# OettlM/STEDM

Hardware: AMD Instinct MI355X
Metric: U-Net denoising steps/sec (32x32x4 latent, bs=64) (higher is better)
Workload: dtype f16; 1 GPU; HER2-style DDIM-50 + CFG 1.5 (rescale 0.7) denoising step, NS32 U-Net (234.6M params, random-init PRNG weights), 32x32x4 latents + 3-ch layout concat, style vector 512; batch_per_gpu=64, global_batch=64, latent=32x32x4, cfg=cond+uncond per step, parallelism=dp1 (independent latents, no in-loop collective)

## Files before the change

include/stedm_hip.h:

```cpp
#ifndef STEDM_HIP_H
#define STEDM_HIP_H

#include <stdint.h>

#ifdef __cplusplus
extern "C" {
#endif

#define STEDM_ABI_VERSION 18

#define STEDM_F16 0
#define STEDM_BF16 1

#define STEDM_CONV_S1 0
#define STEDM_CONV_DOWN 1
#define STEDM_CONV_UP 2
#define STEDM_CONV_UP_SUBPIXEL 3
#define STEDM_CONV_S2D 4

int stedm_abi_version(void);
const char* stedm_last_error(void);
int stedm_device_cus(void);

#define STEDM_F16G_RAW 1
#define STEDM_F16G_NORM 2
#define STEDM_F16G_CONV_OUT16 4
#define STEDM_F16G_S2D 8
#define STEDM_F16G_CAST 16
#define STEDM_F16G_CONV_SRC 32
int stedm_f16_guard_set(void* flag_words);

int stedm_pack_conv_weight(const float* w_oihw, void* w_hi, void* w_lo, int cout, int cin, int ks,
                           int mm_dtype, void* stream);
int stedm_pack_conv_weight_up(const float* w_oihw, void* w_hi, void* w_lo, int cout, int cin, int mm_dtype,
                              void* stream);
int stedm_pack_conv_weight_frag(const float* w_oihw, void* out, int cout, int cin, int ks, int mm_dtype, void* stream);
int stedm_pack_conv_weight_up_frag(const float* w_oihw, void* out, int cout, int cin, int mm_dtype, void* stream);
int stedm_space_to_depth16(const float* x, int C, int B, int H, int W, void* out_hi, void* out_lo, int mm_dtype, void* stream);
int stedm_pack_conv_weight_frag16(const float* w, long sn, long sc, int flip, void* out, int cout, int cin, int ks, int mm_dtype, void* stream);
int stedm_pack_conv_weight_frag16_hl(const float* w, long sn, long sc, int flip, void* out, int cout, int cin, int mm_dtype, void* stream);
int stedm_pack_conv_weight_frag16_hl1(const float* w, long sn, long sc, int flip, void* out, int cout, int cin, int mm_dtype, void* stream);
int stedm_pack_conv_weight_up_frag16_hl(const float* w, void* out, int cout, int cin, int mm_dtype, void* stream);
int stedm_pack_conv_weight_s2d_frag16_hl(const float* w, void* out, int cout, int cin, int mm_dtype, int pad_br, void* stream);
int stedm_pack_conv_weight_s2d_frag(const float* w_oihw, void* out, int cout, int cin, int mm_dtype, int pad_br, void* stream);
int stedm_transpose_f32(const float* in, float* out, int rows, int cols, void* stream);

int stedm_gn_scale_shift(const float* x1, int c1, const float* x2, int c2, int x2_bmod,
                         const float* gamma, const float* beta, float eps, int groups, int B, int HW,
                         float* scale, float* shift, void* stream);

int stedm_gn_nslab(int C, int HW);
int stedm_gn_chan_nslab(int HW);
int stedm_gn_chan_stats(const float* x, int C, int B, int HW, int nslab, float* chan_stats, void* stream);
int stedm_gn_chan_stats16(const float* x, int C, int B, int HW, int nslab, float* chan_stats, void* out_hi, void* out_lo, int mm_dtype,
                          void* stream);
int stedm_gn_apply16c(const float* x1, int c1, const float* cs1, int nslab1, const float* x2, int c2, const float* cs2, int nslab2, int x2_bmod,
                      const float* gamma, const float* beta, float eps, int groups, int act, int B, int HW,
                      void* out_hi, void* out_lo, void* raw_hi, void* raw_lo, int mm_dtype, void* stream);
int stedm_gn_apply16c_mr(const float* x1, int c1, const float* cs1, int nslab1, const float* x2, int c2, const float* cs2, int nslab2, int x2_bmod,
                         const float* gamma, const float* beta, float eps, int groups, int act, int B, int HW,
                         void* out_hi, void* out_lo, void* raw_hi, void* raw_lo, float* mean_rstd, int mm_dtype, void* stream);
int stedm_gn_apply16c_x16(int c1, const float* cs1, int nslab1, const float* x2, int c2, const float* cs2, int nslab2, int x2_bmod,
                          const float* gamma, const float* beta, float eps, int groups, int act, int B, int HW,
                          void* out_hi, void* raw_hi, int mm_dtype, void* stream);
int stedm_gn_stats(const float* x1, int c1, const float* x2, int c2, int x2_bmod, int groups, int B, int HW,
                   double* stats, void* stream);
int stedm_gn_apply16(const float* x1, int c1, const float* x2, int c2, int x2_bmod, const float* gamma,
                     const float* beta, float eps, int groups, int act, const double* stats, int B, int HW,
                     void* out_hi, void* out_lo, int mm_dtype, void* stream);

typedef struct stedm_conv_args {
  const float* src1;
  const float* src2;
  int32_t c1, c2, src2_bmod;
  int32_t B, Hin, Win;
  int32_t mode;
  int32_t ks;
  const float* scale;
  const float* shift;
  int32_t act;
  const void* w_hi;
  const void* w_lo;
  const float* bias;
  const float* emb;
  int32_t emb_bstride;
  const float* res;
  float* out;
  int32_t cout;
  int32_t npass;
  int32_t mm_dtype;
  const void* src16_hi;
  const void* src16_lo;
  int32_t act_out;
  void* out16_hi;
  void* out16_lo;
  const void* w_frag;
  float* chan_stats;
  const void* src16b_hi;
  const void* w_frag_b;
  const float* bias_b;
  int32_t cb;
  float* ws;
  int64_t ws_floats;
  int32_t chan_nslab;
  const void* w_frag16;
  const void* w_frag_b16;
  int32_t pad_br;
  const float* gn_gamma;
  const float* gn_beta;
  float gn_eps;
  int32_t gn_groups;
  int32_t gn_act;
  void* gn_out16;
  float* gn_mr;
  int32_t gn_only;
  void* gn_out16_lo;
  void* qkv_q;
// ... 198 lines not shown
```

stedm_amd/_lib.py:

```python
from __future__ import annotations

import ctypes as C
import os

_HERE = os.path.dirname(os.path.abspath(__file__))
LIB_PATH = os.environ.get("STEDM_HIP_LIB") or os.path.join(_HERE, "libstedm_hip.so")

ABI_VERSION = 18
F16, BF16 = 0, 1
CONV_S1, CONV_DOWN, CONV_UP, CONV_UP_SUBPIXEL, CONV_S2D = 0, 1, 2, 3, 4


class StedmHipError(RuntimeError):
    pass


class ConvArgs(C.Structure):
    _fields_ = [
        ("src1", C.c_void_p), ("src2", C.c_void_p),
        ("c1", C.c_int32), ("c2", C.c_int32), ("src2_bmod", C.c_int32),
        ("B", C.c_int32), ("Hin", C.c_int32), ("Win", C.c_int32),
        ("mode", C.c_int32), ("ks", C.c_int32),
        ("scale", C.c_void_p), ("shift", C.c_void_p),
        ("act", C.c_int32),
        ("w_hi", C.c_void_p), ("w_lo", C.c_void_p), ("bias", C.c_void_p),
        ("emb", C.c_void_p), ("emb_bstride", C.c_int32),
        ("res", C.c_void_p), ("out", C.c_void_p),
        ("cout", C.c_int32), ("npass", C.c_int32), ("mm_dtype", C.c_int32),
        ("src16_hi", C.c_void_p), ("src16_lo", C.c_void_p),
        ("act_out", C.c_int32), ("out16_hi", C.c_void_p), ("out16_lo", C.c_void_p),
        ("w_frag", C.c_void_p), ("chan_stats", C.c_void_p),
        ("src16b_hi", C.c_void_p), ("w_frag_b", C.c_void_p), ("bias_b", C.c_void_p), ("cb", C.c_int32),
        ("ws", C.c_void_p), ("ws_floats", C.c_int64), ("chan_nslab", C.c_int32), ("w_frag16", C.c_void_p), ("w_frag_b16", C.c_void_p), ("pad_br", C.c_int32),
        ("gn_gamma", C.c_void_p), ("gn_beta", C.c_void_p), ("gn_eps", C.c_float), ("gn_groups", C.c_int32), ("gn_act", C.c_int32), ("gn_out16", C.c_void_p), ("gn_mr", C.c_void_p), ("gn_only", C.c_int32),
        ("gn_out16_lo", C.c_void_p),
        ("qkv_q", C.c_void_p), ("qkv_k", C.c_void_p), ("qkv_vt", C.c_void_p),
        ("qkv_T", C.c_int32), ("qkv_Tp", C.c_int32), ("qkv_heads", C.c_int32), ("qkv_qscale", C.c_float),
        ("ln_gamma", C.c_void_p), ("ln_beta", C.c_void_p), ("ln_res", C.c_void_p), ("ln_eps", C.c_float),
        ("out16_stride", C.c_int32),
        ("gn_coop", C.c_void_p), ("gn_coop_epoch", C.c_void_p), ("gn_coop_tmo", C.c_void_p),
    ]


_P, _I, _F = C.c_void_p, C.c_int, C.c_float
SIGNATURES = {
    "stedm_abi_version": (_I, []),
    "stedm_last_error": (C.c_char_p, []),
    "stedm_device_cus": (_I, []),
    "stedm_f16_guard_set": (_I, [_P]),
    "stedm_pack_conv_weight": (_I, [_P, _P, _P, _I, _I, _I, _I, _P]),
    "stedm_pack_conv_weight_up": (_I, [_P, _P, _P, _I, _I, _I, _P]),
    "stedm_pack_conv_weight_frag": (_I, [_P, _P, _I, _I, _I, _I, _P]),
    "stedm_pack_conv_weight_up_frag": (_I, [_P, _P, _I, _I, _I, _P]),
    "stedm_pack_conv_weight_frag16": (_I, [_P, C.c_long, C.c_long, _I, _P, _I, _I, _I, _I, _P]),
    "stedm_pack_conv_weight_frag16_hl": (_I, [_P, C.c_long, C.c_long, _I, _P, _I, _I, _I, _P]),
    "stedm_pack_conv_weight_frag16_hl1": (_I, [_P, C.c_long, C.c_long, _I, _P, _I, _I, _I, _P]),
    "stedm_pack_conv_weight_up_frag16_hl": (_I, [_P, _P, _I, _I, _I, _P]),
    "stedm_pack_conv_weight_s2d_frag16_hl": (_I, [_P, _P, _I, _I, _I, _I, _P]),
    "stedm_pack_conv_weight_s2d_frag": (_I, [_P, _P, _I, _I, _I, _I, _P]),
    "stedm_space_to_depth16": (_I, [_P, _I, _I, _I, _I, _P, _P, _I, _P]),
    "stedm_transpose_f32": (_I, [_P, _P, _I, _I, _P]),
    "stedm_gn_scale_shift": (_I, [_P, _I, _P, _I, _I, _P, _P, _F, _I, _I, _I, _P, _P, _P]),
    "stedm_gn_nslab": (_I, [_I, _I]),
    "stedm_gn_stats": (_I, [_P, _I, _P, _I, _I, _I, _I, _I, _P, _P]),
    "stedm_gn_apply16": (_I, [_P, _I, _P, _I, _I, _P, _P, _F, _I, _I, _P, _I, _I, _P, _P, _I, _P]),
    "stedm_gn_chan_nslab": (_I, [_I]),
    "stedm_gn_chan_stats": (_I, [_P, _I, _I, _I, _I, _P, _P]),
    "stedm_gn_chan_stats16": (_I, [_P, _I, _I, _I, _I, _P, _P, _P, _I, _P]),
    "stedm_gn_apply16c": (_I, [_P, _I, _P, _I, _P, _I, _P, _I, _I, _P, _P, _F, _I, _I, _I, _I, _P, _P, _P, _P, _I, _P]),
    "stedm_gn_apply16c_mr": (_I, [_P, _I, _P, _I, _P, _I, _P, _I, _I, _P, _P, _F, _I, _I, _I, _I, _P, _P, _P, _P, _P, _I, _P]),
    "stedm_conv3x3_tiles_ok": (_I, [_I, _I]),
    "stedm_im2col_rows16": (_I, [_P, _P, _I, _I, _I, _I, _I, _P]),
    "stedm_philox_normal": (_I, [_P, _I, _I, _P, _I, C.c_ulonglong, C.c_uint, _P]),
    "stedm_ddim_mask_blend": (_I, [_P, _P, _P, C.c_long, C.c_long, _P, _P, _P, _P, _P, _I, _I, _I, C.c_long, C.c_ulonglong, _P]),
    "stedm_ddpm_step": (_I, [_P, _P, _P, _P, _I, _I, _P, _P, C.c_long, C.c_long, _P, _P, _P, _P, _I, _I, _I, C.c_long,
                            C.c_ulonglong, C.c_ulonglong, _P]),
    "stedm_gn_apply16c_x16": (_I, [_I, _P, _I, _P, _I, _P, _I, _I, _P, _P, _F, _I, _I, _I, _I, _P, _P, _I, _P]),
    "stedm_conv_igemm": (_I, [C.POINTER(ConvArgs), _P]),
    "stedm_conv_fused_skip_ok": (_I, [C.POINTER(ConvArgs)]),
    "stedm_conv_rs_ok": (_I, [C.POINTER(ConvArgs)]),
    "stedm_conv_in": (_I, [_P, _I, _P, _I, _I, _P, _P, _P, _I, _I, _I, _I, _P, _P]),
    "stedm_conv_out": (_I, [_P, _I, _P, _I, _P, _P, _F, _I, _P, _P, _P, _I, _I, _I, _I, _P]),
    "stedm_time_embed": (_I, [_P, _P, _P, _P, _P, _P, _P, _P, _I, _I, _I, _P]),
    "stedm_time_embed_f32": (_I, [_P, _P, _P, _P, _P, _P, _P, _P, _I, _I, _I, _P]),
    "stedm_emb_proj": (_I, [_P, _P, _P, _P, _I, _I, _I, _P]),
    "stedm_linear": (_I, [_P, _P, _P, _P, _I, _I, _I, _I, _I, _P]),
    "stedm_attn_legacy": (_I, [_P, _P, _I, _I, _I, _I, _P]),
    "stedm_attn_legacy16": (_I, [_P, _I, _P, _I, _I, _I, _I, _I, _P]),
    "stedm_ddim_step": (_I, [_P, _P, _P, _P, _P, _P, _F, _F, _P, _P, _I, _I, _I, _I, _P]),
    "stedm_ddim_step_ex": (_I, [_P, _P, _P, _P, _P, _P, _I, _F, _F, _I, _F, _F, C.c_long, C.c_ulonglong, _P, _P, _P, _P, _I, _I, _I, _I,
                               _P]),
    "stedm_step_advance": (_I, [_P, _I, _P]),
    "stedm_step_set_t": (_I, [_P, _P, _P, _I, _P]),
    "stedm_step_set_t_f32": (_I, [_P, _P, _P, _I, _P]),
    "stedm_dpm_step": (_I, [_P, _P, _P, _P, _P, _P, _P, _F, C.c_long, _P]),
    "stedm_dpm_update": (_I, [_P, _P, _P, _P, _P, C.c_long, _P, _P, _P, _F, _I, C.c_long, _P]),
    "stedm_dpm_threshold": (_I, [_P, C.c_long, _P, _P, _F, _I, C.c_long, _P, _P]),
    "stedm_plms_step": (_I, [_P, _P, _P, _P, _P, _P, _I, _I, _F, _P, _P, C.c_long, _P]),
    "stedm_svit_patch_embed": (_I, [_P, _I, _I, _I, _I, _I, _P, _P, _F, _P, _P, _P, _P, _P, _I, _P]),
    "stedm_svit_patch_ln16": (_I, [_P, _I, _I, _I, _I, _I, _P, _P, _F, _P, _P, _I, _P]),
    "stedm_svit_tok_place": (_I, [_P, _P, _P, _P, _I, _I, _I, _P]),
    "stedm_ln_apply16": (_I, [_P, _P, _P, _F, _P, _P, C.c_long, _I, _I, _P]),
    "stedm_qkv_pack": (_I, [_P, _I, _F, _P, _P, _P, _P, _P, _P, _I, _I, _I, _I, _I, _P]),
    "stedm_lsa_flash": (_I, [_P, _P, _P, _P, _P, _P, _P, _P, _I, _I, _I, _I, _I, _I, _P]),
    "stedm_lsa_flash_drop": (_I, [_P, _P, _P, _P, _P, _P, _P, _P, _I, _I, _I, _I, _I, _I, _F, C.c_ulonglong, C.c_uint, _P]),
    "stedm_dropout_rows": (_I, [_P, _P, _P, _P, _P, C.c_long, _F, C.c_ulonglong, C.c_uint, _I, _P]),
    "stedm_qkv_pack_mx8": (_I, [_P, _I, _F, _P, _P, _P, _P, _P, _P, _I, _I, _I, _I, _I, _P]),
    "stedm_lsa_flash_mx8": (_I, [_P, _P, _P, _P, _P, _P, _P, _I, _I, _I, _I, _I, _P]),
    "stedm_svit_head": (_I, [_P, _I, _I, _I, _I, _P, _P, _P, _F, _P, _P, _P, _I, _P, C.c_long, _P]),
    "stedm_ln_bwd_blocks": (_I, [C.c_long]),
    "stedm_ln_bwd": (_I, [_P, _P, _P, _F, _P, _P, _P, _P, _P, C.c_long, _I, _I, _P]),
    "stedm_geglu_bwd": (_I, [_P, _P, _P, C.c_long, _I, _P]),
    "stedm_geglu16": (_I, [_P, _P, _P, C.c_long, _I, _I, _P]),
    "stedm_agg_reduce": (_I, [_P, _P, _I, _I, _I, _I, _P]),
    "stedm_spatial_rescale": (_I, [_P, _P, _P, _I, _I, _I, _I, _I, _I, _P]),
    "stedm_pack_frag_multi": (_I, [_P, _I, _I, _I, _P]),
    "stedm_swin_patch16": (_I, [_P, C.c_long, C.c_long, C.c_long, C.c_long, _I, _I, _I, _P, _P, _I, _P]),
    "stedm_swin_ln": (_I, [_P, _P, _P, _F, _P, _P, _P, _P, C.c_long, _I, _I, _I, _P]),
    "stedm_swin_ln_gated": (_I, [_P, _P, _P, _F, _P, _P, _P, _P, C.c_long, _I, _I, _P, _I, _I, _P]),
    "stedm_swin_window_attn": (_I, [_P, _P, _P, _P, _P, _P, _P, _I, _I, _I, _I, _I, _I, _I, _I, _I, _P]),
    "stedm_swin_merge16": (_I, [_P, _I, _I, _I, _I, _P, _P, _I, _P]),
    "stedm_swin_rpb": (_I, [_P, _P, _P, _I, _I, _P]),
    "stedm_swin_token_mean": (_I, [_P, _P, _I, _I, _I, _P]),
    "stedm_pack_conv_weight_strided": (_I, [_P, C.c_long, C.c_long, _I, _P, _P, _P, _I, _I, _I, _I, _P]),
    "stedm_gn_fold": (_I, [_P, _I, _I, _P, _I, _I, _I, _I, _I, _F, _P, _P]),
    "stedm_gn_bwd": (_I, [_P, _I, _P, _I, _P, _P, _P, _I, _I, _P, _P, _I, _I, _P, _P, _I, _P, _I, _P, _P, _I, _P, _P, _I, _P]),
    "stedm_gn_bwd_ws_floats": (C.c_long, [_I, _I, _I, _I]),
    "stedm_im2col_t16": (_I, [_P, _P, _I, _I, _I, _I, _I, _I, C.c_long, _P]),
    "stedm_wgrad_to_oihw": (_I, [_P, _P, _I, _I, _I, _I, _I, _I, _I, _P]),
    "stedm_wgrad3x3_plan": (_I, [_I, _I, _I, _I, _I, C.POINTER(C.c_int)]),
# ... 70 lines not shown
```

stedm_amd/csrc/gn.hip:

```cpp
#include <stdlib.h>

#include <type_traits>

#include "common.hpp"
using namespace stedm;

struct GnArgs {
  const float* x1;
  const float* x2;
  int c1, c2, bmod, groups, HW;
  const float* gamma;
  const float* beta;
  float eps;
  float* scale;
  float* shift;
};

template <bool VEC4>
__global__ void __launch_bounds__(256) gn_scale_shift_kernel(GnArgs a) {
  __shared__ float red[4];
  const int b = blockIdx.x / a.groups, g = blockIdx.x % a.groups;
  const int C = a.c1 + a.c2;
  const int cpg = C / a.groups;
  const int cbeg = g * cpg;
// ... 750 lines not shown
    for (int j = 0; j < 8; ++j) h[j] = (T)x[j];
    return __builtin_bit_cast(uint4, h);
  };
  auto over8 = [](uint4 q) { return f16_over2<T>(q.x) | f16_over2<T>(q.y) | f16_over2<T>(q.z) | f16_over2<T>(q.w); };
  auto body = [&](auto tail_c, const int it) {
    constexpr bool TAIL = decltype(tail_c)::value;
    load_adv(vc, it + 2);
    const bool live = !TAIL || it * 256 + (int)threadIdx.x < total;
    const int c = (o_lo + (live ? oc : 0)) * 8;
    float w[8];
    const bool from16 = X16 && c < a.c1;
    if (from16) {
      const V8 h8 = __builtin_bit_cast(V8, va[0]);
#pragma unroll
      for (int j = 0; j < 8; ++j) w[j] = (float)h8[j];
    } else if (PAIR) {
      const bool odd = threadIdx.x & 1;
      const float4 give = odd ? va[0] : va[1];
      float4 got;
      got.x = __shfl_xor(give.x, 1, 64); got.y = __shfl_xor(give.y, 1, 64); got.z = __shfl_xor(give.z, 1, 64); got.w = __shfl_xor(give.w, 1, 64);
      const float4 q0 = odd ? got : va[0], q1 = odd ? va[1] : got;
      w[0] = q0.x; w[1] = q0.y; w[2] = q0.z; w[3] = q0.w; w[4] = q1.x; w[5] = q1.y; w[6] = q1.z; w[7] = q1.w;
    } else {
      w[0] = va[0].x; w[1] = va[0].y; w[2] = va[0].z; w[3] = va[0].w; w[4] = va[1].x; w[5] = va[1].y; w[6] = va[1].z; w[7] = va[1].w;
    }
    const long o = (long)pix * Oall + o_lo + oc;
    if (rh && !from16) {
      const uint4 rq = pack8(w);
      if (maybe_over) bad_raw |= over8(rq);
      if (live) rh[o] = rq;
    }
    const float4 m0 = *reinterpret_cast<const float4*>(tab + c), m1 = *reinterpret_cast<const float4*>(tab + c + 4);
    const float4 s0 = *reinterpret_cast<const float4*>(tab + C + c), s1 = *reinterpret_cast<const float4*>(tab + C + c + 4);
    const float4 b0 = *reinterpret_cast<const float4*>(tab + 2 * C + c), b1 = *reinterpret_cast<const float4*>(tab + 2 * C + c + 4);
    w[0] = (w[0] - m0.x) * s0.x + b0.x; w[1] = (w[1] - m0.y) * s0.y + b0.y; w[2] = (w[2] - m0.z) * s0.z + b0.z; w[3] = (w[3] - m0.w) * s0.w + b0.w;
    w[4] = (w[4] - m1.x) * s1.x + b1.x; w[5] = (w[5] - m1.y) * s1.y + b1.y; w[6] = (w[6] - m1.z) * s1.z + b1.z; w[7] = (w[7] - m1.w) * s1.w + b1.w;
    if (a.act == 1) {
#pragma unroll
      for (int j = 0; j < 8; ++j) w[j] = silu_f(w[j]);
    }
    const uint4 oq = pack8(w);
    if (norm_over) bad_norm |= over8(oq);
    if (live) oh[o] = oq;
    pix += dpix; oc += dq;
    if (oc >= O) { oc -= O; ++pix; }
    va[0] = vb[0]; va[1] = vb[1]; vb[0] = vc[0]; vb[1] = vc[1];
  };
  for (int it = 0; it < nfull; ++it) body(std::false_type{}, it);
  if (nfull * 256 < total) body(std::true_type{}, nfull);
  if (maybe_over) f16_guard_commit(a.ovf, bad_raw, STEDM_F16G_RAW);
  if (norm_over) f16_guard_commit(a.ovf, bad_norm, STEDM_F16G_NORM);
}

extern "C" int stedm_gn_apply16c_mr(const float* x1, int c1, const float* cs1, int nslab1, const float* x2, int c2, const float* cs2, int nslab2, int x2_bmod,
                                    const float* gamma, const float* beta, float eps, int groups, int act, int B, int HW,
                                    void* out_hi, void* out_lo, void* raw_hi, void* raw_lo, float* mean_rstd, int mm_dtype, void* stream);

static int gn_apply16c_launch(GnApplyCArgs a, int B, int mm_dtype, void* stream);

extern "C" int stedm_gn_apply16c_x16(int c1, const float* cs1, int nslab1, const float* x2, int c2, const float* cs2, int nslab2, int x2_bmod,
                                     const float* gamma, const float* beta, float eps, int groups, int act, int B, int HW,
                                     void* out_hi, void* raw_hi, int mm_dtype, void* stream) {
  STEDM_CHECK_ARG(cs1 && out_hi && raw_hi && gamma && beta, "gn_apply16c_x16: null pointer");
  STEDM_CHECK_ARG((x2 != nullptr) == (c2 > 0) && (x2 == nullptr || cs2 != nullptr), "gn_apply16c_x16: x2/c2/cs2 mismatch");
  const int C = c1 + c2;
  STEDM_CHECK_ARG(C % 8 == 0 && c1 % 8 == 0 && c1 > 0 && (size_t)3 * C * sizeof(float) <= 48 * 1024, "gn_apply16c_x16: need c1, c1 + c2 multiples of 8, C <= 4096");
  STEDM_CHECK_ARG(groups > 0 && groups <= 64 && C % groups == 0, "gn_apply16c_x16: need groups <= 64 and C %% groups == 0");
  STEDM_CHECK_ARG(mm_dtype == STEDM_F16 || mm_dtype == STEDM_BF16, "gn_apply16c_x16: bad mm_dtype");
  STEDM_CHECK_ARG(nslab1 > 0 && (x2 == nullptr || nslab2 > 0), "gn_apply16c_x16: nslab1 / nslab2 must be the slot counts of cs1 / cs2");
  GnApplyCArgs a{nullptr, x2, cs1, cs2, c1, c2, x2_bmod, groups, HW, act, nslab1, x2 ? nslab2 : 0, gamma, beta, eps, out_hi, nullptr, raw_hi, nullptr, nullptr,
                 mm_dtype == STEDM_F16 ? f16_guard_flag() : nullptr, raw_hi};
  return gn_apply16c_launch(a, B, mm_dtype, stream);
}

extern "C" int stedm_gn_apply16c(const float* x1, int c1, const float* cs1, int nslab1, const float* x2, int c2, const float* cs2, int nslab2, int x2_bmod,
                                 const float* gamma, const float* beta, float eps, int groups, int act, int B, int HW,
                                 void* out_hi, void* out_lo, void* raw_hi, void* raw_lo, int mm_dtype, void* stream) {
  return stedm_gn_apply16c_mr(x1, c1, cs1, nslab1, x2, c2, cs2, nslab2, x2_bmod, gamma, beta, eps, groups, act, B, HW, out_hi, out_lo, raw_hi, raw_lo,
                              nullptr, mm_dtype, stream);
}

extern "C" int stedm_gn_apply16c_mr(const float* x1, int c1, const float* cs1, int nslab1, const float* x2, int c2, const float* cs2, int nslab2, int x2_bmod,
                                    const float* gamma, const float* beta, float eps, int groups, int act, int B, int HW,
                                    void* out_hi, void* out_lo, void* raw_hi, void* raw_lo, float* mean_rstd, int mm_dtype, void* stream) {
  STEDM_CHECK_ARG(x1 && cs1 && out_hi && gamma && beta, "gn_apply16c: null pointer");
  STEDM_CHECK_ARG((x2 != nullptr) == (c2 > 0) && (x2 == nullptr || cs2 != nullptr), "gn_apply16c: x2/c2/cs2 mismatch");
  const int C = c1 + c2;
  STEDM_CHECK_ARG(C % 4 == 0 && c1 % 4 == 0 && C / 4 <= 1024, "gn_apply16c: channels must be multiples of 4, C <= 4096");
  STEDM_CHECK_ARG(groups > 0 && groups <= 64 && C % groups == 0, "gn_apply16c: need groups <= 64 and C %% groups == 0");
  STEDM_CHECK_ARG(mm_dtype == STEDM_F16 || mm_dtype == STEDM_BF16, "gn_apply16c: bad mm_dtype");
  STEDM_CHECK_ARG(raw_hi || !raw_lo, "gn_apply16c: raw_lo without raw_hi");
  STEDM_CHECK_ARG(nslab1 > 0 && (x2 == nullptr || nslab2 > 0), "gn_apply16c: nslab1 / nslab2 must be the slot counts of cs1 / cs2");
  GnApplyCArgs a{x1, x2, cs1, cs2, c1, c2, x2_bmod, groups, HW, act, nslab1, x2 ? nslab2 : 0, gamma, beta, eps, out_hi, out_lo, raw_hi, raw_lo, mean_rstd,
                 mm_dtype == STEDM_F16 ? f16_guard_flag() : nullptr, nullptr};
  return gn_apply16c_launch(a, B, mm_dtype, stream);
}

static int gn_apply16c_launch(GnApplyCArgs a, int B, int mm_dtype, void* stream) {
  const int C = a.c1 + a.c2, HW = a.HW, groups = a.groups, c1 = a.c1;
  int slab;
  {
    const int want = (128 * 256 + C - 1) / C;
    int per_sample = (HW + want - 1) / want;
    const int need = (768 + B - 1) / B;
    if (per_sample < need) per_sample = need;
    if (per_sample > HW) per_sample = HW;
    slab = (HW + per_sample - 1) / per_sample;
  }
  if (slab < 1) slab = 1;
  if (slab > HW) slab = HW;
  dim3 grid(B, (HW + slab - 1) / slab);
  if (C % 8 == 0 && c1 % 8 == 0 && (size_t)3 * C * sizeof(float) <= 48 * 1024) {
    const size_t lds = (size_t)3 * C * sizeof(float);
    int cb = 0;
    if (grid.y > 1 && HW <= 256) {
      const int cpg = C / groups;
      int unit = cpg;
      while (unit % 8 != 0) unit *= 2;
      for (int t = unit; t <= C / 2; t += unit)
        if (C % t == 0 && c1 % t == 0 && t >= 128 && (long)B * (C / t) >= 768) cb = t;
      if (cb > 0 && (C % cb != 0 || c1 % cb != 0 || cb % unit != 0 || cb / cpg > 64)) cb = 0;
    }
    if (cb > 0) grid = dim3(B, C / cb);
    static const int o8_mode = getenv("STEDM_GN_O8") ? atoi(getenv("STEDM_GN_O8")) : 1;
    const bool o8_ok = !a.out_lo && !a.raw_lo && (cb == 0 || cb % 8 == 0);
    if (o8_ok && ((a.x16 && o8_mode >= 1) || o8_mode >= 2)) {
      static const bool no_pair = getenv("STEDM_GN_NOPAIR") != nullptr;
      const bool pair = C % 16 == 0 && c1 % 16 == 0 && (cb == 0 || cb % 16 == 0) && !no_pair;
#define GN_O8(TT, XX, PP) gn_apply16c_o8_kernel<TT, XX, PP><<<grid, 256, lds, as_stream(stream)>>>(a, slab, cb)
      if (mm_dtype == STEDM_F16) {
        if (a.x16) { if (pair) GN_O8(_Float16, true, true); else GN_O8(_Float16, true, false); }
        else { if (pair) GN_O8(_Float16, false, true); else GN_O8(_Float16, false, false); }
      } else {
        if (a.x16) { if (pair) GN_O8(__bf16, true, true); else GN_O8(__bf16, true, false); }
        else { if (pair) GN_O8(__bf16, false, true); else GN_O8(__bf16, false, false); }
      }
#undef GN_O8
      STEDM_LAUNCH_CHECK();
      return 0;
    }
    if (a.x16) {
      if (mm_dtype == STEDM_F16) gn_apply16c_v8_kernel<_Float16, true><<<grid, 256, lds, as_stream(stream)>>>(a, slab, cb);
      else gn_apply16c_v8_kernel<__bf16, true><<<grid, 256, lds, as_stream(stream)>>>(a, slab, cb);
    } else if (mm_dtype == STEDM_F16) gn_apply16c_v8_kernel<_Float16><<<grid, 256, lds, as_stream(stream)>>>(a, slab, cb);
    else gn_apply16c_v8_kernel<__bf16><<<grid, 256, lds, as_stream(stream)>>>(a, slab, cb);
    STEDM_LAUNCH_CHECK();
    return 0;
  }
  STEDM_CHECK_ARG(!a.x16, "gn_apply16c_x16: the 16-bit source form belongs to the vector kernel");
  if (mm_dtype == STEDM_F16)
    gn_apply16c_kernel<_Float16><<<grid, 256, 0, as_stream(stream)>>>(a, slab);
  else
    gn_apply16c_kernel<__bf16><<<grid, 256, 0, as_stream(stream)>>>(a, slab);
  STEDM_LAUNCH_CHECK();
  return 0;
}
```

stedm_amd/ops.py:

```python
from __future__ import annotations

import ctypes as C
from dataclasses import dataclass
from typing import Optional, Tuple

import torch

from . import _lib
from ._lib import BF16, CONV_DOWN, CONV_S1, CONV_S2D, CONV_UP, CONV_UP_SUBPIXEL, F16, ConvArgs, check, lib


@dataclass(frozen=True)
class Precision:
    mm_dtype: int = F16
    npass: int = 3
    attn_fp8: bool = False

    @staticmethod
    def parse(name: str) -> "Precision":
        table = {"parity": Precision(F16, 3), "parity_bf16": Precision(BF16, 3),
                 "fast": Precision(F16, 1), "f16": Precision(F16, 1), "bf16": Precision(BF16, 1),
                 "fp8": Precision(BF16, 1, True), "bf16+fp8attn": Precision(BF16, 1, True)}
        if name not in table:
            raise ValueError(f"unknown precision {name!r}; choose from {sorted(table)}")
# ... 225 lines not shown

def gn_apply16(x1: torch.Tensor, x2: Optional[torch.Tensor], out_hi: torch.Tensor, out_lo: Optional[torch.Tensor], prec: Precision,
               gamma: Optional[torch.Tensor] = None, beta: Optional[torch.Tensor] = None, eps: float = 1e-5, groups: int = 32,
               act: int = 0, stats: Optional[torch.Tensor] = None, x2_bmod: int = 0) -> None:
    _chk(x1, name="x1")
    B = x1.shape[0]
    HW = x1.numel() // (B * x1.shape[-1])
    c2 = 0 if x2 is None else x2.shape[-1]
    check(lib().stedm_gn_apply16(x1.data_ptr(), x1.shape[-1], _ptr(x2), c2, x2_bmod, _ptr(gamma), _ptr(beta), float(eps), groups,
                                 act, _ptr(stats), B, HW, out_hi.data_ptr(), _ptr(out_lo), prec.mm_dtype, _stream()),
          "stedm_gn_apply16")


def gn_chan_nslab(HW: int) -> int:
    return (HW + 255) // 256


def gn_chan_stats(x: torch.Tensor, out: torch.Tensor) -> None:
    _chk(x, name="x")
    B, C = x.shape[0], x.shape[-1]
    HW = x.numel() // (B * C)
    assert out.dtype == torch.float32 and out.dim() == 4 and out.shape[0] == B and tuple(out.shape[2:]) == (C, 2)
    check(lib().stedm_gn_chan_stats(x.data_ptr(), C, B, HW, out.shape[1], out.data_ptr(), _stream()), "stedm_gn_chan_stats")


def gn_chan_stats16(x: torch.Tensor, out: torch.Tensor, out_hi: torch.Tensor, out_lo: Optional[torch.Tensor], prec: Precision) -> None:
    _chk(x, name="x")
    B, C = x.shape[0], x.shape[-1]
    HW = x.numel() // (B * C)
    assert out.dtype == torch.float32 and out.dim() == 4 and out.shape[0] == B and tuple(out.shape[2:]) == (C, 2)
    assert out_hi.numel() == x.numel() and out_hi.element_size() == 2 and (out_lo is None or out_lo.numel() == x.numel())
    check(lib().stedm_gn_chan_stats16(x.data_ptr(), C, B, HW, out.shape[1], out.data_ptr(), out_hi.data_ptr(), _ptr(out_lo), prec.mm_dtype,
                                      _stream()), "stedm_gn_chan_stats16")


def gn_apply16c(x1: torch.Tensor, cs1: torch.Tensor, x2: Optional[torch.Tensor], cs2: Optional[torch.Tensor], out_hi: torch.Tensor,
                out_lo: Optional[torch.Tensor], prec: Precision, gamma: torch.Tensor, beta: torch.Tensor, eps: float = 1e-5,
                groups: int = 32, act: int = 0, x2_bmod: int = 0, raw: Optional[Tuple[torch.Tensor, Optional[torch.Tensor]]] = None,
                mean_rstd: Optional[torch.Tensor] = None) -> None:
    _chk(x1, name="x1")
    B = x1.shape[0]
    HW = x1.numel() // (B * x1.shape[-1])
    c2 = 0 if x2 is None else x2.shape[-1]
    if mean_rstd is not None:
        assert mean_rstd.dtype == torch.float32 and mean_rstd.is_contiguous() and tuple(mean_rstd.shape) == (B, groups, 2)
    check(lib().stedm_gn_apply16c_mr(x1.data_ptr(), x1.shape[-1], cs1.data_ptr(), cs1.shape[1], _ptr(x2), c2, _ptr(cs2),
                                     0 if cs2 is None else cs2.shape[1], x2_bmod, gamma.data_ptr(),
                                     beta.data_ptr(), float(eps), groups, act, B, HW, out_hi.data_ptr(), _ptr(out_lo),
                                     None if raw is None else raw[0].data_ptr(), None if raw is None else _ptr(raw[1]),
                                     _ptr(mean_rstd), prec.mm_dtype, _stream()), "stedm_gn_apply16c_mr")


def gn_apply16c_x16(c1: int, cs1: torch.Tensor, x2: Optional[torch.Tensor], cs2: Optional[torch.Tensor], out_hi: torch.Tensor, raw_hi: torch.Tensor,
                    prec: Precision, gamma: torch.Tensor, beta: torch.Tensor, eps: float = 1e-5, groups: int = 32, act: int = 0, x2_bmod: int = 0) -> None:
    assert prec.npass == 1 and raw_hi.dtype == torch.int16 and out_hi.dtype == torch.int16 and raw_hi.is_contiguous() and out_hi.is_contiguous()
    B, C = raw_hi.shape[0], raw_hi.shape[-1]
    HW = raw_hi.numel() // (B * C)
    c2 = 0 if x2 is None else x2.shape[-1]
    assert C == c1 + c2 and tuple(out_hi.shape) == tuple(raw_hi.shape)
    check(lib().stedm_gn_apply16c_x16(int(c1), cs1.data_ptr(), cs1.shape[1], _ptr(x2), c2, _ptr(cs2), 0 if cs2 is None else cs2.shape[1], x2_bmod,
                                      gamma.data_ptr(), beta.data_ptr(), float(eps), groups, act, B, HW, out_hi.data_ptr(), raw_hi.data_ptr(),
                                      prec.mm_dtype, _stream()), "stedm_gn_apply16c_x16")


def gn_apply16c_x16_ok(c1: int, c2: int, groups: int = 32) -> bool:
    C = c1 + c2
    return C % 8 == 0 and c1 % 8 == 0 and c1 > 0 and 3 * C * 4 <= 48 * 1024 and 0 < groups <= 64 and C % groups == 0


class LazyPlanes:

    def __init__(self, fn):
        self._fn, self._val = fn, None

    def get(self):
        if self._val is None:
            self._val = self._fn()
        return self._val

    def reset(self):
        self._val = None


class PackPlan:

    def __init__(self, prec: Precision):
        self.prec = prec
        self.items = []
        self._table = None
        self._blocks = 0
        self._fused = frozenset()
        self._rest = None
        self._fresh = None

    def frag(self, w: torch.Tensor, sn: int, sc: int, flip: bool, cout: int, cin: int, ks: int, m16: bool) -> torch.Tensor:
        _chk(w, name="w")
        taps = ks * ks
        if m16:
            assert cin % 32 == 0
            out = torch.empty(((cout + 127) // 128, cin // 32, taps, 8, 64, 8), dtype=torch.int16, device=w.device)
            check(lib().stedm_pack_conv_weight_frag16(w.data_ptr(), sn, sc, int(flip), out.data_ptr(), cout, cin, ks, self.prec.mm_dtype, _stream()),
                  "stedm_pack_conv_weight_frag16")
        else:
            assert cin % 16 == 0
            out = torch.empty(((cout + 127) // 128, cin // 16, taps, 4, 64, 8), dtype=torch.int16, device=w.device)
            check(lib().stedm_pack_conv_weight_strided(w.data_ptr(), sn, sc, int(flip), None, None, out.data_ptr(), cout, cin, ks, self.prec.mm_dtype,
                                                       _stream()), "stedm_pack_conv_weight_strided")
        self.items.append((w, sn, sc, int(flip), cout, cin, taps, int(m16), out))
        self._table = None
        self._rest = None
        self._fresh = None
        return out

    def frag_oihw(self, w4: torch.Tensor, m16: bool) -> torch.Tensor:
        cout, cin, ks, _ = w4.shape
# ... 1041 lines not shown
```

Baseline: 164.7 steps/s.

## Add CFG-pair GroupNorm apply kernel sharing skip-channel loads across cond/uncond halves

Result: no change. 164.5 steps/s (-0.1%).

```diff
diff --git a/include/stedm_hip.h b/include/stedm_hip.h
--- a/include/stedm_hip.h
+++ b/include/stedm_hip.h
@@ -7,7 +7,7 @@
 extern "C" {
 #endif
 
-#define STEDM_ABI_VERSION 18
+#define STEDM_ABI_VERSION 19
 
 #define STEDM_F16 0
 #define STEDM_BF16 1
@@ -63,6 +63,9 @@
 int stedm_gn_apply16c_x16(int c1, const float* cs1, int nslab1, const float* x2, int c2, const float* cs2, int nslab2, int x2_bmod,
                           const float* gamma, const float* beta, float eps, int groups, int act, int B, int HW,
                           void* out_hi, void* raw_hi, int mm_dtype, void* stream);
+int stedm_gn_apply16c_x16_form(int c1, const float* cs1, int nslab1, const float* x2, int c2, const float* cs2, int nslab2, int x2_bmod,
+                               const float* gamma, const float* beta, float eps, int groups, int act, int B, int HW,
+                               void* out_hi, void* raw_hi, int mm_dtype, int form, void* stream);
 int stedm_gn_stats(const float* x1, int c1, const float* x2, int c2, int x2_bmod, int groups, int B, int HW,
                    double* stats, void* stream);
 int stedm_gn_apply16(const float* x1, int c1, const float* x2, int c2, int x2_bmod, const float* gamma,
diff --git a/stedm_amd/_lib.py b/stedm_amd/_lib.py
--- a/stedm_amd/_lib.py
+++ b/stedm_amd/_lib.py
@@ -6,7 +6,7 @@
 _HERE = os.path.dirname(os.path.abspath(__file__))
 LIB_PATH = os.environ.get("STEDM_HIP_LIB") or os.path.join(_HERE, "libstedm_hip.so")
 
-ABI_VERSION = 18
+ABI_VERSION = 19
 F16, BF16 = 0, 1
 CONV_S1, CONV_DOWN, CONV_UP, CONV_UP_SUBPIXEL, CONV_S2D = 0, 1, 2, 3, 4
 
@@ -76,6 +76,7 @@
     "stedm_ddpm_step": (_I, [_P, _P, _P, _P, _I, _I, _P, _P, C.c_long, C.c_long, _P, _P, _P, _P, _I, _I, _I, C.c_long,
                             C.c_ulonglong, C.c_ulonglong, _P]),
     "stedm_gn_apply16c_x16": (_I, [_I, _P, _I, _P, _I, _P, _I, _I, _P, _P, _F, _I, _I, _I, _I, _P, _P, _I, _P]),
+    "stedm_gn_apply16c_x16_form": (_I, [_I, _P, _I, _P, _I, _P, _I, _I, _P, _P, _F, _I, _I, _I, _I, _P, _P, _I, _I, _P]),
     "stedm_conv_igemm": (_I, [C.POINTER(ConvArgs), _P]),
     "stedm_conv_fused_skip_ok": (_I, [C.POINTER(ConvArgs)]),
     "stedm_conv_rs_ok": (_I, [C.POINTER(ConvArgs)]),
diff --git a/stedm_amd/csrc/gn.hip b/stedm_amd/csrc/gn.hip
--- a/stedm_amd/csrc/gn.hip
+++ b/stedm_amd/csrc/gn.hip
@@ -826,15 +826,198 @@
   if (norm_over) f16_guard_commit(a.ovf, bad_norm, STEDM_F16G_NORM);
 }
 
+template <typename T>
+__device__ __forceinline__ uint4 gn_pack8(const float (&x)[8]) {
+  typedef T V8 __attribute__((ext_vector_type(8)));
+  V8 h;
+#pragma unroll
+  for (int j = 0; j < 8; ++j) h[j] = (T)x[j];
+  return __builtin_bit_cast(uint4, h);
+}
+template <typename T>
+__device__ __forceinline__ unsigned gn_over8(uint4 q) { return f16_over2<T>(q.x) | f16_over2<T>(q.y) | f16_over2<T>(q.z) | f16_over2<T>(q.w); }
+
+template <typename T>
+__device__ __forceinline__ uint4 gn_norm8(const float (&x)[8], const float* tm, const float* ts, const float* tb, const int act) {
+  float w[8];
+  const float4 m0 = *reinterpret_cast<const float4*>(tm), m1 = *reinterpret_cast<const float4*>(tm + 4);
+  const float4 s0 = *reinterpret_cast<const float4*>(ts), s1 = *reinterpret_cast<const float4*>(ts + 4);
+  const float4 b0 = *reinterpret_cast<const float4*>(tb), b1 = *reinterpret_cast<const float4*>(tb + 4);
+  w[0] = (x[0] - m0.x) * s0.x + b0.x; w[1] = (x[1] - m0.y) * s0.y + b0.y; w[2] = (x[2] - m0.z) * s0.z + b0.z; w[3] = (x[3] - m0.w) * s0.w + b0.w;
+  w[4] = (x[4] - m1.x) * s1.x + b1.x; w[5] = (x[5] - m1.y) * s1.y + b1.y; w[6] = (x[6] - m1.z) * s1.z + b1.z; w[7] = (x[7] - m1.w) * s1.w + b1.w;
+  if (act == 1) {
+#pragma unroll
+    for (int j = 0; j < 8; ++j) w[j] = silu_f(w[j]);
+  }
+  return gn_pack8<T>(w);
+}
+
+template <typename T>
+__global__ void __launch_bounds__(256) gn_apply16c_o8_kernel_cfg(GnApplyCArgs a, int slab, int cb) {
+  typedef T V8 __attribute__((ext_vector_type(8)));
+  __shared__ double dsu[256], dsq[256];
+  __shared__ float lmean[2][64], lrstd[2][64];
+  extern __shared__ __attribute__((aligned(16))) float tab[];
+  const int sl = blockIdx.y;
+  const int C = a.c1 + a.c2, Oall = C >> 3;
+  const int cpg = C / a.groups;
+  const int c_lo = cb > 0 ? sl * cb : 0, c_n = cb > 0 ? cb : C;
+  const int O = c_n >> 3, o_lo = c_lo >> 3;
+  const int O1 = (min(c_lo + c_n, a.c1) - min(c_lo, a.c1)) >> 3;
+  const bool two = cb == 0;
+  const bool skip_run = cb > 0 && c_lo >= a.c1;
+  const int hp = (a.HW + 1) >> 1;
+  const int bA = skip_run ? (int)blockIdx.x % a.bmod : (int)blockIdx.x;
+  const int bB = (cb == 0 || skip_run) ? bA + a.bmod : bA;
+  const int px0 = cb == 0 ? sl * slab : skip_run ? ((int)blockIdx.x / a.bmod) * hp : 0;
+  const int px1 = cb == 0 ? min(a.HW, px0 + slab) : skip_run ? min(a.HW, px0 + hp) : a.HW;
+  if (px0 >= px1) return;
+  const int b2 = bA % a.bmod;
+  const float* p2 = a.x2 + (long)b2 * a.HW * a.c2;
+  const T* p16 = reinterpret_cast<const T*>(a.x16);
+  const int OB = two ? O1 : 0x7fffffff;
+  const int V = O + (two ? O1 : 0);
+  const int total = (px1 - px0) * V;
+  const int gsh = ((a.c1 + cpg - 1) / cpg) * cpg;
+  uint4* ohA = reinterpret_cast<uint4*>(a.out_hi) + (long)bA * a.HW * Oall;
+  uint4* ohB = reinterpret_cast<uint4*>(a.out_hi) + (long)bB * a.HW * Oall;
+  uint4* rhA = reinterpret_cast<uint4*>(a.raw_hi) + (long)bA * a.HW * Oall;
+  uint4* rhB = reinterpret_cast<uint4*>(a.raw_hi) + (long)bB * a.HW * Oall;
+  const long dAB = (long)(bB - bA) * a.HW * Oall;
+  int pix = px0 + (int)threadIdx.x / V, voc = (int)threadIdx.x % V;
+  int lpx = pix, lvoc = voc;
+  const int dpix = 256 / V, dq = 256 % V;
+  float4 va[2], vb[2], vc[2];
+  const int nfull = total / 256;
+  auto load_adv = [&](float4 (&dst)[2], int it) {
+    const bool ok = it * 256 + (int)threadIdx.x < total;
+    const int px = ok ? lpx : px0, vo = ok ? lvoc : 0;
+    const bool sub = vo >= OB;
+    const int c = (o_lo + vo - (sub ? O1 : 0)) * 8;
+    const bool h16 = c < a.c1;
+    const int bs = bA + ((sub && h16) ? a.bmod : 0);
+    const float* f32 = p2 + (long)px * a.c2 + (c - a.c1);
+    const char* s0 = h16 ? reinterpret_cast<const char*>(p16 + ((long)bs * a.HW + px) * C + c)
+                         : reinterpret_cast<const char*>(f32) - ((ok && (threadIdx.x & 1)) ? 16 : 0);
+    const char* s1 = h16 ? s0 : s0 + (ok ? 32 : 16);
+    dst[0] = *reinterpret_cast<const float4*>(s0);
+    dst[1] = *reinterpret_cast<const float4*>(s1);
+    lpx += dpix; lvoc += dq;
+    if (lvoc >= V) { lvoc -= V; ++lpx; }
+  };
+  load_adv(va, 0);
+  load_adv(vb, 1);
+  bool maybe_over = false, norm_over = false;
+  unsigned bad_raw = 0u, bad_norm = 0u;
+  {
+    const int g_lo = c_lo / cpg, ng = c_n / cpg;
+    const int L = 256 / ng;
+    const int gl = threadIdx.x / L, l = threadIdx.x % L, g = g_lo + gl;
+    int big_any = 0;
+    for (int s = 0; s < (two ? 2 : 1); ++s) {
+      const int bs = s ? bB : bA;
+      const bool on = gl < ng && (s == 0 || g * cpg < a.c1);
+      double su = 0.0, sq = 0.0;
+      int big = 0;
+      if (on) {
+        const int nmax = a.nslab1 > a.nslab2 ? a.nslab1 : a.nslab2;
+        const int n = cpg * nmax;
+        for (int e = l; e < n; e += L) {
+          const int k = e / cpg, c = g * cpg + (e - k * cpg);
+          if (c < a.c1) {
+            if (k < a.nslab1) { const float* p = a.cs1 + (((long)bs * a.nslab1 + k) * a.c1 + c) * 2; su += (double)p[0]; sq += (double)p[1]; big |= !(p[1] < STEDM_F16_SQ_SAFE); }
+          } else if (k < a.nslab2) {
+            const float* p = a.cs2 + (((long)b2 * a.nslab2 + k) * a.c2 + (c - a.c1)) * 2; su += (double)p[0]; sq += (double)p[1]; big |= !(p[1] < STEDM_F16_SQ_SAFE);
+          }
+        }
+      }
+      dsu[threadIdx.x] = su; dsq[threadIdx.x] = sq;
+      big_any |= __syncthreads_or(big);
+      if (on && l == 0) {
+        double s_ = 0.0, q_ = 0.0;
+        for (int i = 0; i < L; ++i) { s_ += dsu[threadIdx.x + i]; q_ += dsq[threadIdx.x + i]; }
+        const double inv_n = 1.0 / ((double)cpg * a.HW);
+        const double mean = s_ * inv_n;
+        double var = q_ * inv_n - mean * mean;
+        var = var > 0.0 ? var : 0.0;
+        lmean[s][g] = (float)mean;
+        lrstd[s][g] = (float)(1.0 / sqrt(var + (double)a.eps));
+      }
+      __syncthreads();
+    }
+    maybe_over = big_any != 0 && a.ovf != nullptr && __is_same(T, _Float16);
+    int nb = 0;
+    const bool guard = a.ovf != nullptr && __is_same(T, _Float16);
+    const float rn = sqrtf((float)cpg * (float)a.HW);
+    for (int c = c_lo + threadIdx.x; c < c_lo + c_n; c += 256) {
+      const int gc = c / cpg;
+      const float gmc = a.gamma[c], btc = a.beta[c];
+      tab[c] = lmean[0][gc];
+      tab[C + c] = lrstd[0][gc] * gmc;
+      tab[2 * C + c] = btc;
+      if (two) { const int s = gc * cpg < a.c1 ? 1 : 0; tab[3 * C + c] = lmean[s][gc]; tab[4 * C + c] = lrstd[s][gc] * gmc; }
+      if (guard) nb |= !(rn * fabsf(gmc) + fabsf(btc) < 65504.f);
+    }
+    norm_over = __syncthreads_or(nb) != 0;
+  }
+  auto body = [&](auto tail_c, const int it) {
+    constexpr bool TAIL = decltype(tail_c)::value;
+    const bool live = !TAIL || it * 256 + (int)threadIdx.x < total;
+    const int vo = live ? voc : 0;
+    const bool sub = vo >= OB;
+    const int oc = vo - (sub ? O1 : 0);
+    const int c = (o_lo + oc) * 8;
+    const bool from16 = c < a.c1;
+    const long o = (long)pix * Oall + o_lo + oc;
+    float w[8];
+    if (from16) {
+      const V8 h8 = __builtin_bit_cast(V8, va[0]);
+#pragma unroll
+      for (int j = 0; j < 8; ++j) w[j] = (float)h8[j];
+    } else {
+      const bool odd = threadIdx.x & 1;
+      const float4 give = odd ? va[0] : va[1];
+      float4 got;
+      got.x = __shfl_xor(give.x, 1, 64); got.y = __shfl_xor(give.y, 1, 64); got.z = __shfl_xor(give.z, 1, 64); got.w = __shfl_xor(give.w, 1, 64);
+      const float4 q0 = odd ? got : va[0], q1 = odd ? va[1] : got;
+      w[0] = q0.x; w[1] = q0.y; w[2] = q0.z; w[3] = q0.w; w[4] = q1.x; w[5] = q1.y; w[6] = q1.z; w[7] = q1.w;
+      const uint4 rq = gn_pack8<T>(w);
+      if (maybe_over) bad_raw |= gn_over8<T>(rq);
+      if (live) { rhA[o] = rq; rhB[o] = rq; }
+    }
+    const bool hB = from16 && sub;
+    const int to = hB ? 3 * C : 0;
+    const uint4 qa = gn_norm8<T>(w, tab + to + c, tab + to + C + c, tab + 2 * C + c, a.act);
+    if (norm_over) bad_norm |= gn_over8<T>(qa);
+    if (from16) {
+      if (live) ohA[o + (hB ? dAB : 0)] = qa;
+    } else {
+      uint4 qb = qa;
+      if (c < gsh) {
+        qb = gn_norm8<T>(w, tab + 3 * C + c, tab + 4 * C + c, tab + 2 * C + c, a.act);
+        if (norm_over) bad_norm |= gn_over8<T>(qb);
+      }
+      if (live) { ohA[o] = qa; ohB[o] = qb; }
+    }
+    pix += dpix; voc += dq;
+    if (voc >= V) { voc -= V; ++pix; }
+    va[0] = vb[0]; va[1] = vb[1]; vb[0] = vc[0]; vb[1] = vc[1];
+  };
+  for (int it = 0; it < nfull; ++it) { load_adv(vc, it + 2); body(std::false_type{}, it); }
+  if (nfull * 256 < total) { load_adv(vc, nfull + 2); body(std::true_type{}, nfull); }
+  if (maybe_over) f16_guard_commit(a.ovf, bad_raw, STEDM_F16G_RAW);
+  if (norm_over) f16_guard_commit(a.ovf, bad_norm, STEDM_F16G_NORM);
+}
+
 extern "C" int stedm_gn_apply16c_mr(const float* x1, int c1, const float* cs1, int nslab1, const float* x2, int c2, const float* cs2, int nslab2, int x2_bmod,
                                     const float* gamma, const float* beta, float eps, int groups, int act, int B, int HW,
                                     void* out_hi, void* out_lo, void* raw_hi, void* raw_lo, float* mean_rstd, int mm_dtype, void* stream);
 
-static int gn_apply16c_launch(GnApplyCArgs a, int B, int mm_dtype, void* stream);
-
-extern "C" int stedm_gn_apply16c_x16(int c1, const float* cs1, int nslab1, const float* x2, int c2, const float* cs2, int nslab2, int x2_bmod,
-                                     const float* gamma, const float* beta, float eps, int groups, int act, int B, int HW,
-                                     void* out_hi, void* raw_hi, int mm_dtype, void* stream) {
+static int gn_apply16c_launch(GnApplyCArgs a, int B, int mm_dtype, void* stream, int form = 1);
+
+extern "C" int stedm_gn_apply16c_x16_form(int c1, const float* cs1, int nslab1, const float* x2, int c2, const float* cs2, int nslab2, int x2_bmod,
+                                          const float* gamma, const float* beta, float eps, int groups, int act, int B, int HW,
+                                          void* out_hi, void* raw_hi, int mm_dtype, int form, void* stream) {
   STEDM_CHECK_ARG(cs1 && out_hi && raw_hi && gamma && beta, "gn_apply16c_x16: null pointer");
   STEDM_CHECK_ARG((x2 != nullptr) == (c2 > 0) && (x2 == nullptr || cs2 != nullptr), "gn_apply16c_x16: x2/c2/cs2 mismatch");
   const int C = c1 + c2;
@@ -842,9 +1025,16 @@
   STEDM_CHECK_ARG(groups > 0 && groups <= 64 && C % groups == 0, "gn_apply16c_x16: need groups <= 64 and C %% groups == 0");
   STEDM_CHECK_ARG(mm_dtype == STEDM_F16 || mm_dtype == STEDM_BF16, "gn_apply16c_x16: bad mm_dtype");
   STEDM_CHECK_ARG(nslab1 > 0 && (x2 == nullptr || nslab2 > 0), "gn_apply16c_x16: nslab1 / nslab2 must be the slot counts of cs1 / cs2");
+  STEDM_CHECK_ARG(form >= 0 && form <= 2, "gn_apply16c_x16: form must be 0 (host decides), 1 (per sample) or 2 (CFG pair)");
   GnApplyCArgs a{nullptr, x2, cs1, cs2, c1, c2, x2_bmod, groups, HW, act, nslab1, x2 ? nslab2 : 0, gamma, beta, eps, out_hi, nullptr, raw_hi, nullptr, nullptr,
                  mm_dtype == STEDM_F16 ? f16_guard_flag() : nullptr, raw_hi};
-  return gn_apply16c_launch(a, B, mm_dtype, stream);
+  return gn_apply16c_launch(a, B, mm_dtype, stream, form);
+}
+
+extern "C" int stedm_gn_apply16c_x16(int c1, const float* cs1, int nslab1, const float* x2, int c2, const float* cs2, int nslab2, int x2_bmod,
+                                     const float* gamma, const float* beta, float eps, int groups, int act, int B, int HW,
+                                     void* out_hi, void* raw_hi, int mm_dtype, void* stream) {
+  return stedm_gn_apply16c_x16_form(c1, cs1, nslab1, x2, c2, cs2, nslab2, x2_bmod, gamma, beta, eps, groups, act, B, HW, out_hi, raw_hi, mm_dtype, 0, stream);
 }
 
 extern "C" int stedm_gn_apply16c(const float* x1, int c1, const float* cs1, int nslab1, const float* x2, int c2, const float* cs2, int nslab2, int x2_bmod,
@@ -870,19 +1060,21 @@
   return gn_apply16c_launch(a, B, mm_dtype, stream);
 }
 
-static int gn_apply16c_launch(GnApplyCArgs a, int B, int mm_dtype, void* stream) {
-  const int C = a.c1 + a.c2, HW = a.HW, groups = a.groups, c1 = a.c1;
-  int slab;
-  {
-    const int want = (128 * 256 + C - 1) / C;
-    int per_sample = (HW + want - 1) / want;
-    const int need = (768 + B - 1) / B;
-    if (per_sample < need) per_sample = need;
-    if (per_sample > HW) per_sample = HW;
-    slab = (HW + per_sample - 1) / per_sample;
-  }
+static int gn_apply16c_slab(int C, int B, int HW) {
+  const int want = (128 * 256 + C - 1) / C;
+  int per_sample = (HW + want - 1) / want;
+  const int need = (768 + B - 1) / B;
+  if (per_sample < need) per_sample = need;
+  if (per_sample > HW) per_sample = HW;
+  int slab = (HW + per_sample - 1) / per_sample;
   if (slab < 1) slab = 1;
   if (slab > HW) slab = HW;
+  return slab;
+}
+
+static int gn_apply16c_launch(GnApplyCArgs a, int B, int mm_dtype, void* stream, int form) {
+  const int C = a.c1 + a.c2, HW = a.HW, groups = a.groups, c1 = a.c1;
+  const int slab = gn_apply16c_slab(C, B, HW);
   dim3 grid(B, (HW + slab - 1) / slab);
   if (C % 8 == 0 && c1 % 8 == 0 && (size_t)3 * C * sizeof(float) <= 48 * 1024) {
     const size_t lds = (size_t)3 * C * sizeof(float);
@@ -896,6 +1088,18 @@
       if (cb > 0 && (C % cb != 0 || c1 % cb != 0 || cb % unit != 0 || cb / cpg > 64)) cb = 0;
     }
     if (cb > 0) grid = dim3(B, C / cb);
+    const bool cfg_ok = a.x16 && a.x2 && B >= 2 && B % 2 == 0 && a.bmod == B / 2 && C % 16 == 0 && c1 % 16 == 0 && (cb == 0 || cb % 16 == 0) &&
+                        (size_t)5 * C * sizeof(float) <= 48 * 1024;
+    STEDM_CHECK_ARG(form != 2 || cfg_ok, "gn_apply16c_x16: the CFG-pair form needs an even B, x2_bmod == B / 2 and c1, c1 + c2 multiples of 16 (C <= 2432)");
+    if (cfg_ok && form != 1) {
+      const int pslab = cb > 0 ? slab : gn_apply16c_slab(C, B / 2, HW);
+      const dim3 pgrid = cb > 0 ? grid : dim3(B / 2, (HW + pslab - 1) / pslab);
+      const size_t plds = (size_t)5 * C * sizeof(float);
+      if (mm_dtype == STEDM_F16) gn_apply16c_o8_kernel_cfg<_Float16><<<pgrid, 256, plds, as_stream(stream)>>>(a, pslab, cb);
+      else gn_apply16c_o8_kernel_cfg<__bf16><<<pgrid, 256, plds, as_stream(stream)>>>(a, pslab, cb);
+      STEDM_LAUNCH_CHECK();
+      return 0;
+    }
     static const int o8_mode = getenv("STEDM_GN_O8") ? atoi(getenv("STEDM_GN_O8")) : 1;
     const bool o8_ok = !a.out_lo && !a.raw_lo && (cb == 0 || cb % 8 == 0);
     if (o8_ok && ((a.x16 && o8_mode >= 1) || o8_mode >= 2)) {
diff --git a/stedm_amd/ops.py b/stedm_amd/ops.py
--- a/stedm_amd/ops.py
+++ b/stedm_amd/ops.py
@@ -301,15 +301,16 @@
 
 
 def gn_apply16c_x16(c1: int, cs1: torch.Tensor, x2: Optional[torch.Tensor], cs2: Optional[torch.Tensor], out_hi: torch.Tensor, raw_hi: torch.Tensor,
-                    prec: Precision, gamma: torch.Tensor, beta: torch.Tensor, eps: float = 1e-5, groups: int = 32, act: int = 0, x2_bmod: int = 0) -> None:
+                    prec: Precision, gamma: torch.Tensor, beta: torch.Tensor, eps: float = 1e-5, groups: int = 32, act: int = 0, x2_bmod: int = 0,
+                    form: int = 0) -> None:
     assert prec.npass == 1 and raw_hi.dtype == torch.int16 and out_hi.dtype == torch.int16 and raw_hi.is_contiguous() and out_hi.is_contiguous()
     B, C = raw_hi.shape[0], raw_hi.shape[-1]
     HW = raw_hi.numel() // (B * C)
     c2 = 0 if x2 is None else x2.shape[-1]
     assert C == c1 + c2 and tuple(out_hi.shape) == tuple(raw_hi.shape)
-    check(lib().stedm_gn_apply16c_x16(int(c1), cs1.data_ptr(), cs1.shape[1], _ptr(x2), c2, _ptr(cs2), 0 if cs2 is None else cs2.shape[1], x2_bmod,
-                                      gamma.data_ptr(), beta.data_ptr(), float(eps), groups, act, B, HW, out_hi.data_ptr(), raw_hi.data_ptr(),
-                                      prec.mm_dtype, _stream()), "stedm_gn_apply16c_x16")
+    check(lib().stedm_gn_apply16c_x16_form(int(c1), cs1.data_ptr(), cs1.shape[1], _ptr(x2), c2, _ptr(cs2), 0 if cs2 is None else cs2.shape[1], x2_bmod,
+                                           gamma.data_ptr(), beta.data_ptr(), float(eps), groups, act, B, HW, out_hi.data_ptr(), raw_hi.data_ptr(),
+                                           prec.mm_dtype, int(form), _stream()), "stedm_gn_apply16c_x16_form")
 
 
 def gn_apply16c_x16_ok(c1: int, c2: int, groups: int = 32) -> bool:
```
